# jinhojsk515/spmm

Measured on AMD Instinct MI355X. Metric: pretrain molecules/sec, higher is better.
Workload: dtype bf16; 1 GPU; SPMM pretrain step, text 12 layers (fusion at 6) + PV 6 layers, H=768, 12 heads, queue 36864, train mode (dropout 0.1), fwd+bwd+clip+AdamW+EMA; global_batch=128, seq_len=128, parallelism=dp1, schedule=eager launches on three HIP streams, packed text rows

## Files before the change

include/spmm_hip.h:

```cpp
#ifndef SPMM_HIP_H
#define SPMM_HIP_H

#include <stdint.h>

#ifdef __HIPCC__
#include <hip/hip_runtime.h>
typedef hipStream_t spmm_stream_t;
#else
typedef void* spmm_stream_t;
#endif

#ifdef __cplusplus
extern "C" {
#endif

int spmm_version(void);
const char* spmm_last_error(void);

#define SPMM_EPI_BF16 0
#define SPMM_EPI_GELU 1
#define SPMM_EPI_F32 2
#define SPMM_EPI_F32_ATOMIC 3
#define SPMM_EPI_GELU_GRAD 4
#define SPMM_EPI_F32_ACC 5
// ... 72 lines not shown
int spmm_beam_step_until(const float* logits, long ldl, int N, int k, int V, int Lmax, int F, int t, const int* t_ptr, int t_off,
                         int* tokens, float* cur_p, float* fin_p, int* fin_len, int* fin_tok, int* fin_n, unsigned char* done,
                         int* anc, int anc_ld, int* ids_out, int* parent_out, int* n_done, const int* mol, const int* rowmap,
                         int need, spmm_stream_t stream);

int spmm_beam_step_sampled(const float* logits, long ldl, int N, int k, int V, int Lmax, int F, int t, const int* t_ptr, int t_off,
                           int* tokens, float* cur_p, float* fin_p, int* fin_len, int* fin_tok, int* fin_n, unsigned char* done,
                           int* anc, int anc_ld, int* ids_out, int* parent_out, int* n_done, const int* mol, const int* rowmap,
                           const float* noise, long ldn, spmm_stream_t stream);

int spmm_gumbel_noise(const uint64_t* seed_ptr, uint64_t salt, int N, int k, int V, int Lmax, int t, const int* t_ptr, int t_off,
                      const int* mol, long mol_base, float* out, long ldo, spmm_stream_t stream);

int spmm_logit_warp(const float* lc, const float* lu, long ld, int R, int V, float w, float temperature, int top_k, float top_p,
                    int min_keep, float* out, long ldo, spmm_stream_t stream);

#define SPMM_SYNTAX_MASKED (-1e30f)
int spmm_smiles_mask(float* logits, float* logits2, long ld, int R, int V, const int* tokens, long tok_ld, int hist_rows, int k,
                     const int* mol, int Lmax, int t, const int* t_ptr, int t_off, int t_last, const int* table, int* state_out,
                     spmm_stream_t stream);

int spmm_wordpiece(const unsigned char* blob, const long* offsets, int N, int gap, const unsigned char* head, int head_len,
                   const int* table, int table_words, int max_chars, int max_pieces, int unk_id, int sep_id, int pad_id,
                   int* ids, long ld, int* lens, int* status, spmm_stream_t stream);

int spmm_sbs_step(const float* logits, long ldl, const float* noise, long ldn, int G, int W, int V, int Lmax, int t, const int* t_ptr,
                  int t_off, const float* phi_in, const float* gum_in, const unsigned char* fin_in, const int* len_in,
                  const int* tokens_in, const int* anc_in, float* phi_out, float* gum_out, unsigned char* fin_out, int* len_out,
                  int* tokens_out, int* anc_out, int anc_ld, int* ids_out, int* parent_out, int* open_out, unsigned int* ws,
                  spmm_stream_t stream);

int spmm_kv_prefill(const void* K, const void* V, long ld, long src_rows, const int* row0, const int* len, const int* dst_row, int E,
                    void* Kc, void* Vc, int R, int nH, int Lmax, spmm_stream_t stream);

int spmm_embed_ln_fwd(int mode, const int* ids, const float* word, const float* pos, const float* type0, const float* pv_x,
                      const float* pv_mask, const float* pv_w, const float* pv_b, const float* pv_cls,
                      const float* pv_masktok, int src_mod, const float* gamma, const float* beta, void* y, void* zout,
                      float* mean, float* rstd, long nseq, int L, int H, float eps, float dropout_p,
                      const uint64_t* seed_ptr, uint64_t salt, spmm_stream_t stream);
int spmm_embed_bwd(int mode, const void* dz, const int* ids, const float* pv_x, const float* pv_mask, int src_mod,
                   float* dword, float* dpos, float* dtype0, float* d_w, float* d_b, float* d_cls, float* d_masktok,
                   long nseq, int L, int H, spmm_stream_t stream);

int spmm_transpose_bf16(const void* in, long ldi, void* out, long ldo, int R, int C, int Rpad, float* colsum,
                        spmm_stream_t stream);
int spmm_cast_transpose(const float* in, void* out, void* outT, int R, int C, spmm_stream_t stream);
long spmm_cast_transpose_desc_bytes(void);
int spmm_cast_transpose_multi(const void* descs_dev, int ndesc, int total_tiles, spmm_stream_t stream);
int spmm_cast_f32_bf16(const float* in, void* out, long n, spmm_stream_t stream);
int spmm_cast_bf16_f32(const void* in, float* out, long n, spmm_stream_t stream);
int spmm_acc_rows(float* dst, long ldd, const void* src, long lds, const long* idx, long rows, int H, int atomic,
                  spmm_stream_t stream);
int spmm_gather_rows(void* dst, const void* src, const long* idx, long rows, int H, spmm_stream_t stream);

int spmm_gather_rows2(void* dst, const void* srcA, const void* srcB, const long* idx, long rows, int H, spmm_stream_t stream);
int spmm_add_rows_bf16(void* dst, const long* idx, const void* src, long rows, int H, spmm_stream_t stream);
int spmm_zero_bytes(void* p, long nbytes, spmm_stream_t stream);
int spmm_zero_rows(void* p, long rows, long row_bytes, long stride_bytes, spmm_stream_t stream);
int spmm_gelu_bwd(const void* dz, const void* pre, void* out, long n, spmm_stream_t stream);
int spmm_pack_plan(const int* mask, int B, int Lt, int M, int* lens32, int* row0_32, long* row0_64, long* rows, long* gidx2,
                   long* gidx4, long* inv, long* idx_m, int* bad, spmm_stream_t stream);
int spmm_fusion_plan(const long* neg, const int* lens32, const int* row0_32, int B, int Lt, int Lp, int M,
                     long* idx6, long* neg_rows, long* idx_top, int* small32, spmm_stream_t stream);

int spmm_l2norm_fwd(const float* x, long ldx, float* y, float* nrm, void* a3, void* w3, void* yT, long ldt, int rows, int E,
                    spmm_stream_t stream);
int spmm_l2norm_bwd(const float* dy, const float* y, const float* nrm, const float* gscale, void* dx, int rows, int E,
                    spmm_stream_t stream);
int spmm_ita_rows(const float* S, const float* SM, long ldj, int nrows, int B, int J, const float* alpha_ptr,
                  const float* temp_ptr, void* dS, long ldd, int Jpad, float* losses, int loss_slot, float* dtemp,
                  int* nan_flag, spmm_stream_t stream);
int spmm_sample_neg(const float* S, long ldj, int B, const long* forced, const uint64_t* seed_ptr, uint64_t salt, long* out,
                    long out_offset, spmm_stream_t stream);
int spmm_lm_loss(const float* logits, const float* logits_m, long ldl, const int* ids, long nseq, int L, int V,
                 const float* alpha_ptr, int* n_nonpad_ws, const float* gscale, void* dlogits, long ldd, int Vpad,
                 float* losses, int loss_slot, spmm_stream_t stream);
int spmm_s2s_loss(const float* logits, long ldl, const int* ids, const long* row_of, long rows, long nseq, int L, int V,
                  int* n_label_ws, const float* gscale, void* dlogits, long ldd, int Vpad, float* losses, int loss_slot,
                  spmm_stream_t stream);
int spmm_lm_score(const void* y, long ldy, const void* Wd, long ldw, const float* bias, const int* ids, const long* row_of, long rows,
                  long nseq, int L, int V, int H, const int* seq_row0, const int* seq_len, float* tok_lp, float* seq_lp, int* seq_n,
                  spmm_stream_t stream);
int spmm_itm_head(const void* xa, long stride_a, const void* xb, long stride_b, int H, const float* W, const float* bias,
                  int n, int B, const float* gscale, float* losses, int loss_slot, float* logits_out, void* dxa, void* dxb,
                  float* dW, float* db, int do_bwd, int x_is_f32, spmm_stream_t stream);
int spmm_task_head(const void* A, long lda, int B, int W, const float* W2, const float* b2, int C, int kind, const void* target,
                   const float* gscale, float* logits, float* loss, void* dA, long ldda, float* dW2, float* db2, int do_bwd,
                   spmm_stream_t stream);
int spmm_s2p_append(const void* y, long ldy, const float* w3, const float* b3, const float* pe_w, const float* pe_b, const float* pos,
                    const float* type0, const float* gamma, const float* beta, float eps, float* pred, long ldp, void* xcache,
                    long rows, int H, int n_props, int i, spmm_stream_t stream);
int spmm_mpm_head(const void* h, int Lp, int H, const float* w, const float* bias, const float* target, const float* mask,
                  int B, int* n_keep_ws, const float* gscale, float* losses, int loss_slot, float* pred_out, void* dh,
                  float* dw, float* db, int do_bwd, int x_is_f32, spmm_stream_t stream);
int spmm_rows_linear(const void* x, int x_is_bf16, long ldx, const float* W, const float* bias, float* out, long ldo, long rows,
                     int N, int K, int act, spmm_stream_t stream);
long spmm_sim_topk_workspace_bytes(int Q, long n, int k);
int spmm_sim_topk(const float* q, long ldq, const float* f, long ldf, long base, int Q, long n, int E, int k, float* scores, long* index,
                  int merge, const float* cut_scores, const long* cut_index, void* workspace, long workspace_bytes, spmm_stream_t stream);
int spmm_centroid_assign(const float* f, long ldf, const float* c, long ldc, long c0, long n, int Kc, int E, float* best, int* assign,
                         int merge, const int* prev, int* changed, spmm_stream_t stream);
long spmm_cluster_group_workspace_bytes(long n, int K);
int spmm_cluster_group(const int* assign, long n, int K, int* counts, long* offsets, int* members, int* outside, void* workspace,
                       long workspace_bytes, spmm_stream_t stream);
long spmm_cluster_centroids_workspace_bytes(long n, int K, int E);
int spmm_cluster_centroids(const float* f, long ldf, long n, int E, const float* best, const int* counts, const long* offsets,
// ... 21 lines not shown
```

spmm_amd/csrc/rowops.hip:

```cpp
#include "common.h"
#include <stdlib.h>
#include "../../include/spmm_hip.h"

namespace {

constexpr int MAXC = 4;

struct RowVec {
  float v[MAXC][4];
};

__device__ __forceinline__ void load_row_bf16(const bf16* __restrict__ p, int H, int lane, RowVec& r) {
#pragma unroll
  for (int i = 0; i < MAXC; ++i) {
    const int c = (lane + 64 * i) * 4;
    if (c < H) {
      const bf16x4 t = *(const bf16x4*)(p + c);
      r.v[i][0] = (float)t[0]; r.v[i][1] = (float)t[1]; r.v[i][2] = (float)t[2]; r.v[i][3] = (float)t[3];
    } else {
      r.v[i][0] = r.v[i][1] = r.v[i][2] = r.v[i][3] = 0.f;
    }
  }
}
__device__ __forceinline__ void store_row_bf16(bf16* __restrict__ p, int H, int lane, const RowVec& r) {
// ... 433 lines not shown
    const uint32_t rowkey = drop_rowkey(seed_mix(p.seed_ptr, p.salt), (uint64_t)row);
#pragma unroll
    for (int i = 0; i < MAXC; ++i) {
      const int c = (lane + 64 * i) * 4;
      if (c < p.H) {
        bool k[4];
        drop_keep4(rowkey, c, p.thresh16, k);
#pragma unroll
        for (int j = 0; j < 4; ++j) o.v[i][j] = k[j] ? o.v[i][j] * p.dscale : 0.f;
      }
    }
  }
  store_row_bf16(p.y + row * p.H, p.H, lane, o);
  if (p.zout) store_row_bf16(p.zout + row * p.H, p.H, lane, z);
  if (p.mean_o && lane == 0) { p.mean_o[row] = mean; p.rstd_o[row] = rstd; }
}

struct EmbedBwdP {
  const bf16* dz; const int* ids; const float* pv_x; const float* pv_mask; int src_mod;
  float* dword; float* dpos; float* dtype0; float* d_w; float* d_b; float* d_cls; float* d_masktok;
  long nseq; int L, H, mode;
};
__global__ __launch_bounds__(256) void embed_bwd_kernel(EmbedBwdP p) {
  const int l = blockIdx.x;
  const long s_per = (p.nseq + gridDim.y - 1) / gridDim.y;
  const long s_beg = blockIdx.y * s_per, s_end = min(p.nseq, s_beg + s_per);
  for (int c = threadIdx.x; c < p.H; c += 256) {
    float acc = 0.f, accw = 0.f, accb = 0.f, accm = 0.f;
    for (long s = s_beg; s < s_end; ++s) {
      const long row = s * p.L + l;
      const float g = (float)p.dz[row * p.H + c];
      acc += g;
      if (p.mode == 0) {
        const int id = p.ids[row];
        if (id != 0) atomicAdd(p.dword + (long)id * p.H + c, g);
      } else if (l > 0) {
        const long src = (s % p.src_mod) * (p.L - 1) + (l - 1);
        const float m = p.pv_mask[src];
        accw += g * (1.f - m) * p.pv_x[src];
        accb += g * (1.f - m);
        accm += g * m;
      }
    }
    atomicAdd(p.dpos + (long)l * p.H + c, acc);
    atomicAdd(p.dtype0 + c, acc);
    if (p.mode == 1) {
      if (l == 0) {
        atomicAdd(p.d_cls + c, acc);
      } else {
        atomicAdd(p.d_w + c, accw);
        atomicAdd(p.d_b + c, accb);
        atomicAdd(p.d_masktok + c, accm);
      }
    }
  }
}

__global__ __launch_bounds__(256) void transpose_bf16_kernel(const bf16* __restrict__ in, long ldi, bf16* __restrict__ out,
                                                             long ldo, int R, int C, int Rpad, float* __restrict__ colsum) {
  __shared__ bf16 tile[64][66];
  const int r0 = blockIdx.y * 64, c0 = blockIdx.x * 64;
  const int tx = threadIdx.x & 63, ty = threadIdx.x >> 6;
  float cs = 0.f;
#pragma unroll
  for (int i = 0; i < 16; ++i) {
    const int r = r0 + ty * 16 + i, c = c0 + tx;
    const bf16 v = (r < R && c < C) ? in[(long)r * ldi + c] : (bf16)0.f;
    tile[ty * 16 + i][tx] = v;
    cs += (float)v;
  }
  if (colsum) {
    __shared__ float part[4][64];
    part[ty][tx] = cs;
    __syncthreads();
    if (ty == 0 && c0 + tx < C) atomicAdd(colsum + c0 + tx, part[0][tx] + part[1][tx] + part[2][tx] + part[3][tx]);
  } else {
    __syncthreads();
  }
#pragma unroll
  for (int i = 0; i < 16; ++i) {
    const int c = c0 + ty * 16 + i, r = r0 + tx;
    if (c < C && r < Rpad) out[(long)c * ldo + r] = tile[tx][ty * 16 + i];
  }
}

__global__ __launch_bounds__(256) void cast_transpose_kernel(const float* __restrict__ in, bf16* __restrict__ out,
                                                             bf16* __restrict__ outT, int R, int C) {
  __shared__ bf16 tile[64][66];
  const int r0 = blockIdx.y * 64, c0 = blockIdx.x * 64;
  const int tx = threadIdx.x & 63, ty = threadIdx.x >> 6;
#pragma unroll
  for (int i = 0; i < 16; ++i) {
    const int r = r0 + ty * 16 + i, c = c0 + tx;
    bf16 v = (bf16)0.f;
    if (r < R && c < C) {
      v = (bf16)in[(long)r * C + c];
      if (out) out[(long)r * C + c] = v;
    }
    tile[ty * 16 + i][tx] = v;
  }
  __syncthreads();
  if (outT) {
#pragma unroll
    for (int i = 0; i < 16; ++i) {
      const int c = c0 + ty * 16 + i, r = r0 + tx;
      if (c < C && r < R) outT[(long)c * R + r] = tile[tx][ty * 16 + i];
// ... 148 lines not shown
  return SPMM_OK;
}

extern "C" int spmm_embed_ln_fwd(int mode, const int* ids, const float* word, const float* pos, const float* type0,
                                 const float* pv_x, const float* pv_mask, const float* pv_w, const float* pv_b,
                                 const float* pv_cls, const float* pv_masktok, int src_mod, const float* gamma,
                                 const float* beta, void* y, void* zout, float* mean, float* rstd, long nseq, int L, int H,
                                 float eps, float dropout_p, const uint64_t* seed_ptr, uint64_t salt, hipStream_t stream) {
  SPMM_CHECK_SHAPE(nseq > 0 && L > 0 && H > 0 && H % 4 == 0 && H <= 1024, "spmm_embed_ln_fwd: nseq=%ld L=%d H=%d (need 0 < H <= 1024, H%%4==0)", nseq, L, H);
  SPMM_CHECK_SHAPE(mode >= 0 && mode <= 2, "spmm_embed_ln_fwd: unknown mode %d", mode);
  SPMM_CHECK_SHAPE(pos && type0 && gamma && beta && y, "spmm_embed_ln_fwd: null pos / type0 / gamma / beta / y");
  SPMM_CHECK_SHAPE((mean == nullptr) == (rstd == nullptr), "spmm_embed_ln_fwd: mean and rstd come together");
  SPMM_CHECK_SHAPE(mode == 0 ? (ids && word) : mode == 2 ? (pv_x != nullptr) : (pv_x && pv_mask && pv_w && pv_b && pv_cls && pv_masktok && src_mod > 0),
                   "spmm_embed_ln_fwd: missing inputs for mode %d", mode);
  SPMM_CHECK_SHAPE(dropout_p == 0.f || seed_ptr, "spmm_embed_ln_fwd: dropout needs a device seed");
  EmbedP p = {};
  p.ids = ids; p.word = word; p.pos = pos; p.type0 = type0; p.pv_x = pv_x; p.pv_mask = pv_mask; p.pv_w = pv_w; p.pv_b = pv_b;
  p.pv_cls = pv_cls; p.pv_masktok = pv_masktok; p.src_mod = src_mod; p.gamma = gamma; p.beta = beta; p.y = (bf16*)y;
  p.zout = (bf16*)zout; p.mean_o = mean; p.rstd_o = rstd; p.nseq = nseq; p.L = L; p.H = H; p.mode = mode; p.eps = eps;
  p.thresh16 = (uint32_t)(dropout_p * 65536.f + 0.5f); p.dscale = 1.f / (1.f - dropout_p); p.seed_ptr = seed_ptr; p.salt = salt;
  hipLaunchKernelGGL(embed_ln_fwd_kernel, dim3((nseq * L + 3) / 4), dim3(256), 0, stream, p);
  SPMM_LAUNCH_CHECK("spmm_embed_ln_fwd");
  return SPMM_OK;
}

extern "C" int spmm_embed_step_ln_fwd(const int* ids, int pos_index, const int* pos_ptr, const float* word, const float* pos, const float* type0,
                                      const float* gamma, const float* beta, void* y, long rows, int H, float eps,
                                      hipStream_t stream) {
  SPMM_CHECK_SHAPE(rows > 0 && pos_index >= 0 && H % 4 == 0 && H <= 1024, "spmm_embed_step_ln_fwd: rows=%ld pos=%d H=%d", rows, pos_index, H);
  SPMM_CHECK_SHAPE(ids && word && pos && type0 && gamma && beta && y, "spmm_embed_step_ln_fwd: null argument");
  EmbedP p = {};
  p.ids = ids; p.word = word; p.pos = pos; p.type0 = type0; p.gamma = gamma; p.beta = beta; p.y = (bf16*)y;
  p.nseq = rows; p.L = 1; p.H = H; p.mode = 0; p.eps = eps; p.pos0 = pos_index; p.pos_ptr = pos_ptr; p.dscale = 1.f;
  hipLaunchKernelGGL(embed_ln_fwd_kernel, dim3((rows + 3) / 4), dim3(256), 0, stream, p);
  SPMM_LAUNCH_CHECK("spmm_embed_step_ln_fwd");
  return SPMM_OK;
}

extern "C" int spmm_embed_bwd(int mode, const void* dz, const int* ids, const float* pv_x, const float* pv_mask, int src_mod,
                              float* dword, float* dpos, float* dtype0, float* d_w, float* d_b, float* d_cls,
                              float* d_masktok, long nseq, int L, int H, hipStream_t stream) {
  SPMM_CHECK_SHAPE(nseq > 0 && L > 0 && H > 0, "spmm_embed_bwd: nseq=%ld L=%d H=%d", nseq, L, H);
  SPMM_CHECK_SHAPE(mode == 0 || mode == 1, "spmm_embed_bwd: mode %d (0 = text, 1 = PV; inputs_embeds has no backward)", mode);
  SPMM_CHECK_SHAPE(dz && dpos && dtype0, "spmm_embed_bwd: null dz / dpos / dtype0");
  SPMM_CHECK_SHAPE(mode != 0 || (ids && dword), "spmm_embed_bwd: mode 0 needs ids and dword");
  SPMM_CHECK_SHAPE(mode != 1 || (pv_x && pv_mask && d_w && d_b && d_cls && d_masktok), "spmm_embed_bwd: mode 1 needs pv_x, pv_mask, d_w, d_b, d_cls and d_masktok");
  SPMM_CHECK_SHAPE(mode != 1 || src_mod > 0, "spmm_embed_bwd: mode 1 needs src_mod > 0, got src_mod=%d", src_mod);
  EmbedBwdP p = {(const bf16*)dz, ids, pv_x, pv_mask, src_mod, dword, dpos, dtype0, d_w, d_b, d_cls, d_masktok, nseq, L, H, mode};
  hipLaunchKernelGGL(embed_bwd_kernel, dim3(L, nseq >= 32 ? 16 : 1), dim3(256), 0, stream, p);
  SPMM_LAUNCH_CHECK("spmm_embed_bwd");
  return SPMM_OK;
}

namespace {
__global__ __launch_bounds__(256) void segment_sum_kernel(const bf16* __restrict__ src, const int* __restrict__ start,
                                                          const int* __restrict__ list, bf16* __restrict__ out, long W) {
  const int u = blockIdx.y;
  const long c = ((long)blockIdx.x * 256 + threadIdx.x) * 8;
  if (c >= W) return;
  const int k0 = start[u], k1 = start[u + 1];
  float acc[8] = {0.f, 0.f, 0.f, 0.f, 0.f, 0.f, 0.f, 0.f};
  for (int k = k0; k < k1; ++k) {
    const bf16x8 v = *(const bf16x8*)(src + (long)list[k] * W + c);
#pragma unroll
    for (int e = 0; e < 8; ++e) acc[e] += (float)v[e];
  }
  bf16x8 o;
#pragma unroll
  for (int e = 0; e < 8; ++e) o[e] = (bf16)acc[e];
  *(bf16x8*)(out + (long)u * W + c) = o;
}
}

extern "C" int spmm_segment_sum_bf16(const void* src, const int* start, const int* list, void* out, int U, long W, hipStream_t stream) {
  SPMM_CHECK_SHAPE(U > 0 && U <= 65535 && W > 0 && W % 8 == 0, "spmm_segment_sum_bf16: U=%d W=%ld (W %% 8 == 0)", U, W);
  SPMM_CHECK_SHAPE(src && start && list && out, "spmm_segment_sum_bf16: null src / start / list / out");
  hipLaunchKernelGGL(segment_sum_kernel, dim3((unsigned)((W / 8 + 255) / 256), U), dim3(256), 0, stream, (const bf16*)src, start, list,
                     (bf16*)out, W);
  SPMM_LAUNCH_CHECK("spmm_segment_sum_bf16");
  return SPMM_OK;
}

extern "C" int spmm_transpose_bf16(const void* in, long ldi, void* out, long ldo, int R, int C, int Rpad, float* colsum,
                                   hipStream_t stream) {
  SPMM_CHECK_SHAPE(R > 0 && C > 0 && Rpad >= R && ldo >= Rpad, "spmm_transpose_bf16: R=%d C=%d Rpad=%d ldo=%ld", R, C, Rpad, ldo);
  SPMM_CHECK_SHAPE(ldi >= C, "spmm_transpose_bf16: ldi=%ld is shorter than a row of C=%d", ldi, C);
  SPMM_CHECK_SHAPE(in && out, "spmm_transpose_bf16: null in / out");
  hipLaunchKernelGGL(transpose_bf16_kernel, dim3((C + 63) / 64, (Rpad + 63) / 64), dim3(256), 0, stream, (const bf16*)in, ldi,
                     (bf16*)out, ldo, R, C, Rpad, colsum);
  SPMM_LAUNCH_CHECK("spmm_transpose_bf16");
  return SPMM_OK;
}

extern "C" int spmm_cast_transpose(const float* in, void* out, void* outT, int R, int C, hipStream_t stream) {
  SPMM_CHECK_SHAPE(R > 0 && C > 0, "spmm_cast_transpose: R=%d C=%d", R, C);
  SPMM_CHECK_SHAPE(in && (out || outT), "spmm_cast_transpose: null in, or neither out nor outT");
  hipLaunchKernelGGL(cast_transpose_kernel, dim3((C + 63) / 64, (R + 63) / 64), dim3(256), 0, stream, in, (bf16*)out, (bf16*)outT, R, C);
  SPMM_LAUNCH_CHECK("spmm_cast_transpose");
  return SPMM_OK;
}

extern "C" long spmm_cast_transpose_desc_bytes(void) { return sizeof(CtDesc); }
extern "C" int spmm_cast_transpose_multi(const void* descs_dev, int ndesc, int total_tiles, hipStream_t stream) {
  SPMM_CHECK_SHAPE(ndesc > 0 && total_tiles > 0, "spmm_cast_transpose_multi: ndesc=%d tiles=%d", ndesc, total_tiles);
  hipLaunchKernelGGL(cast_transpose_multi_kernel, dim3(total_tiles), dim3(256), 0, stream, (const CtDesc*)descs_dev, ndesc);
  SPMM_LAUNCH_CHECK("spmm_cast_transpose_multi");
// ... 37 lines not shown
```

spmm_amd/ops.py:

```python
import ctypes
import os

import torch

from ._lib import lib

EPI_BF16, EPI_GELU, EPI_F32, EPI_F32_ATOMIC, EPI_GELU_GRAD, EPI_F32_ACC, EPI_GELU_DERIV, EPI_MUL = range(8)
BF16 = torch.bfloat16


_DRY_RUN = False
_dry_log = []


def _p(t):
    return None if t is None else ctypes.c_void_p(t.data_ptr())


def _st():
    if _DRY_RUN:
        return None
    return ctypes.c_void_p(torch.cuda.current_stream().cuda_stream)


# ... 169 lines not shown

def ln_bwd(dy, z, mean, rstd, gamma, dz, *, dy2=None, dx=None, dgamma=None, dbeta=None, dropout_p=0.0, seed=None, salt=0,
           drop_on_dy=False, dxsum=None, rows_dev=None, beta_from_y=None):
    rows, H = dy.shape
    _call("spmm_ln_bwd", _p(dy), _p(dy2), _p(z), _p(mean), _p(rstd), _p(gamma), _p(dz), _p(dx), _p(dgamma), _p(dbeta),
               rows, H, float(dropout_p), _p(seed), salt, int(drop_on_dy), _p(dxsum), _p(rows_dev), _p(beta_from_y), _st())
    return dz


def embed_ln_fwd(mode, y, *, nseq, L, H, pos, type0, gamma, beta, ids=None, word=None, pv_x=None, pv_mask=None, pv_w=None,
                 pv_b=None, pv_cls=None, pv_masktok=None, src_mod=1, zout=None, mean=None, rstd=None, eps=1e-12,
                 dropout_p=0.0, seed=None, salt=0):
    _call("spmm_embed_ln_fwd", mode, _p(ids), _p(word), _p(pos), _p(type0), _p(pv_x), _p(pv_mask), _p(pv_w), _p(pv_b),
               _p(pv_cls), _p(pv_masktok), src_mod, _p(gamma), _p(beta), _p(y), _p(zout), _p(mean), _p(rstd), nseq, L, H,
               float(eps), float(dropout_p), _p(seed), salt, _st())
    return y


def embed_bwd(mode, dz, *, nseq, L, H, dpos, dtype0, ids=None, dword=None, pv_x=None, pv_mask=None, src_mod=1, d_w=None,
              d_b=None, d_cls=None, d_masktok=None):
    _call("spmm_embed_bwd", mode, _p(dz), _p(ids), _p(pv_x), _p(pv_mask), src_mod, _p(dword), _p(dpos), _p(dtype0),
               _p(d_w), _p(d_b), _p(d_cls), _p(d_masktok), nseq, L, H, _st())


def transpose_bf16(x, out, *, Rpad=None, colsum=None):
    R, C = x.shape
    Rpad = out.shape[1] if Rpad is None else Rpad
    _call("spmm_transpose_bf16", _p(x), _row_stride(x), _p(out), _row_stride(out), R, C, Rpad, _p(colsum), _st())
    return out


def cast_transpose(w32, out, outT):
    R, C = w32.shape
    _call("spmm_cast_transpose", _p(w32), _p(out), _p(outT), R, C, _st())


def cast_transpose_multi(descs_dev, ndesc, total_tiles):
    _call("spmm_cast_transpose_multi", _p(descs_dev), ndesc, total_tiles, _st())


def cast_f32_bf16(x, out):
    _call("spmm_cast_f32_bf16", _p(x), _p(out), x.numel(), _st())
    return out


def cast_bf16_f32(x, out):
    _call("spmm_cast_bf16_f32", _p(x), _p(out), x.numel(), _st())
    return out


def acc_rows(dst, src, *, idx=None, atomic=False):
    rows, H = src.shape
    _call("spmm_acc_rows", _p(dst), _row_stride(dst), _p(src), _row_stride(src), _p(idx), rows, H, int(atomic), _st())


def gather_rows(dst, src, idx):
    rows, H = dst.shape
    _call("spmm_gather_rows", _p(dst), _p(src), _p(idx), rows, H, _st())
    return dst


SRC_B = 1 << 40


def gather_rows2(dst, srcA, idx, srcB=None):
    rows, H = dst.shape
    assert idx.dtype == torch.int64 and idx.numel() >= rows and dst.is_contiguous() and srcA.is_contiguous() and (srcB is None or srcB.is_contiguous())
    assert dst.dtype == BF16 and srcA.dtype == BF16 and srcA.shape[1] == H and (srcB is None or (srcB.dtype == BF16 and srcB.shape[1] == H))
    _call("spmm_gather_rows2", _p(dst), _p(srcA), _p(srcB), _p(idx), rows, H, _st())
    return dst


def add_rows_bf16(dst, idx, src):
    rows, H = src.shape
    assert dst.dtype == BF16 and src.dtype == BF16 and idx.dtype == torch.int64 and dst.is_contiguous() and src.is_contiguous() and dst.shape[1] == H
    _call("spmm_add_rows_bf16", _p(dst), _p(idx), _p(src), rows, H, _st())
    return dst


def zero_(t):
    n = t.numel() * t.element_size()
    if n == 0:
        return t
    if not t.is_contiguous():
        es = t.element_size()
        if t.dim() == 2 and t.stride(1) == 1 and (t.shape[1] * es) % 16 == 0 and (t.stride(0) * es) % 16 == 0 and t.data_ptr() % 16 == 0:
            _call("spmm_zero_rows", _p(t), t.shape[0], t.shape[1] * es, t.stride(0) * es, _st())
            return t
        return t.zero_()
    if n % 16 or t.data_ptr() % 16:
        return t.zero_()
    _call("spmm_zero_bytes", _p(t), n, _st())
    return t


def gelu_bwd(dz, pre, out=None):
    assert dz.dtype == BF16 and pre.dtype == BF16 and dz.is_contiguous() and pre.is_contiguous() and dz.shape == pre.shape
    out = torch.empty_like(dz) if out is None else out
    _call("spmm_gelu_bwd", _p(dz), _p(pre), _p(out), dz.numel(), _st())
    return out


def pack_plan(mask32, M, bad):
    B, Lt = mask32.shape
    dev = mask32.device
    alloc = torch.zeros if _DRY_RUN else torch.empty
# ... 533 lines not shown
```

spmm_amd/options.py:

```python
from __future__ import annotations

import dataclasses
import os
from dataclasses import dataclass

_ENV = {
    "pack_text": ("SPMM_PACK_TEXT", lambda s: s != "0"),
    "cls_only_top": ("SPMM_CLS_ONLY_TOP", lambda s: s != "0"),
    "multi_stream": ("SPMM_STREAMS", lambda s: s != "1"),
    "wgrad_stream": ("SPMM_WGRAD_STREAM", lambda s: s != "0"),
    "pv_wgrad_inline": ("SPMM_PV_WGRAD_INLINE", int),
    "ln_from_y": ("SPMM_LN_FROM_Y", lambda s: s != "0"),
    "resid_fp32": ("SPMM_RESID_FP32", lambda s: s == "1"),
    "fused_xattn": ("SPMM_FUSED_XATTN", lambda s: {"0": "off", "1": "all"}.get(s, s)),
    "grad_overlap": ("SPMM_GRAD_OVERLAP", lambda s: s != "0"),
    "grad_wire": ("SPMM_GRAD_WIRE", str),
    "nt_under_comm": ("SPMM_NT_UNDER_COMM", str),
    "force_dist": ("SPMM_FORCE_DIST", lambda s: s == "1"),
    "dp_four_streams": ("SPMM_DP_FOUR_STREAMS", lambda s: s != "0"),
    "probe_streams": ("SPMM_PROBE_STREAMS", lambda s: s != "0"),
    "schedule_check": ("SPMM_SCHEDULE_CHECK", lambda s: s != "0"),
}


@dataclass
class EngineOptions:
    pack_text: bool = True
    cls_only_top: bool = True
    multi_stream: bool = True
    wgrad_stream: bool = True
    pv_wgrad_inline: int = 4
    ln_from_y: bool = True
    fused_xattn: str = "nograd"
    resid_fp32: bool = False
    grad_overlap: bool = True
    grad_wire: str = "fp32"
    nt_under_comm: str = "auto"
    force_dist: bool = False
    dp_four_streams: bool = True
    schedule_check: bool = True
    probe_streams: bool = False

    @classmethod
    def from_env(cls, **overrides) -> "EngineOptions":
        kw = {}
        for field, (var, parse) in _ENV.items():
            if var in os.environ:
                kw[field] = parse(os.environ[var])
        kw.update(overrides)
        o = cls(**kw)
        if isinstance(o.fused_xattn, bool):
            o.fused_xattn = "all" if o.fused_xattn else "off"
        if o.fused_xattn not in ("off", "nograd", "all"):
            raise ValueError(f"fused_xattn must be off, nograd or all, not {o.fused_xattn!r}")
        if o.grad_wire not in ("fp32", "bf16"):
            raise ValueError(f"grad_wire must be fp32 or bf16, not {o.grad_wire!r}")
        if o.nt_under_comm not in ("tiles", "persistent", "auto"):
            raise ValueError(f"nt_under_comm must be tiles, persistent or auto, not {o.nt_under_comm!r}")
        return o

    def replace(self, **kw) -> "EngineOptions":
        return dataclasses.replace(self, **kw)
```

spmm_amd/step.py:

```python
from __future__ import annotations

from typing import Callable, Optional, Tuple

import torch

from . import ops, streams
from .engine import STREAM_TOKENS_MAX, BF, LOSS_ITA, LOSS_ITM, LOSS_MLM, LOSS_MPM, Batch, Engine, Group, KVSource, SelfKV, _ceil


class PretrainStep(Engine):
    def _s6_forward_cls(self, B, Lt, M, pk, mask32, neg, y1, y2, prop_embeds, text_embeds, save):
        cfg = self.cfg
        ct = cfg.text
        H, Lp, f, n = ct.hidden_size, cfg.n_props + 1, ct.fusion_layer, ct.num_hidden_layers
        fp = ops.fusion_plan(neg, pk, Lp)
        o_tp = 3 * B * Lp
        o_lm = o_tp + 2 * M
        o_12 = o_lm + B * Lt
        o_8 = o_12 + B * Lp
        Rcap = fp["Rcap"]
        X6 = ops.gather_rows2(self._new(Rcap, H), y1, fp["idx6"], y2)
        src_pv = KVSource(prop_embeds.view(B * Lp, H), B, Lp).preset(4 * B, fp["start_p"], fp["list_p"])
        src_text = KVSource(text_embeds, B, Lt, row0=pk["row0"], length=pk["len"], pack_idx=pk["rows"]).preset(4 * B, fp["start_t"], fp["list_t"])
        ar = fp["ar"]
# ... 257 lines not shown

        if aux is not None:
            aux.update(prop_embeds=prop_embeds, text_embeds=text_embeds, prop_embeds_m=prop_embeds_m, text_embeds_m=text_embeds_m,
                       prop_feat=feats["property_proj"][0], text_feat=feats["text_proj"][0], prop_feat_m=feats["property_proj_m"][0],
                       text_feat_m=feats["text_proj_m"][0], sim_i2t=S_text[:B], sim_t2i=S_prop[B:2 * B], sim_i2t_m=S_text[2 * B:3 * B],
                       vl_output=vl_logits, mlm_output=logits.view(B, Lt, -1)[:, :-1], logits_m=logits_m.view(B, Lt, -1)[:, :-1],
                       pred=pred, prop_neg_idx=neg[:B], text_neg_idx=neg[B:], mpm_mask=mpm_mask,
                       prop_embeds_causal=prop_embeds_causal)
        if save:
            self.tape = dict(B=B, Lt=Lt, pk=pk, M=M, Mn=Mn, src_text=src_text, src_pv=src_pv, neg_rows=neg_rows, cls_text=cls_text, itm_text=itm_text,
                             prop=prop, mpm_mask=mpm_mask, ids32=ids32, ids2=ids2, esv1=esv1, g1=g1, tape1=tape1,
                             esv2=esv2, g2=g2, tape2=tape2, feats=feats, dfeat=dfeat, neg=neg, g6=g6, tape6=tape6, ypv=ypv_h,
                             ytext=ytext, logits=logits, logits_m=logits_m, lmsv=lmsv, mpmsv=mpmsv, S6=S6 if cls_top else None)
        return self.losses[:4]

    def backward(self):
        T = self.tape
        if T is None:
            raise RuntimeError("backward() without a taped forward()")
        self.pre_backward_wait()
        cfg, P = self.cfg, self.P
        ct, cp = cfg.text, cfg.prop
        H, E, Lp, f, n = ct.hidden_size, cfg.embed_dim, cfg.n_props + 1, ct.fusion_layer, ct.num_hidden_layers
        B, Lt = T["B"], T["Lt"]
        gs = self.gscale
        scratch = self.loss_scratch
        pk, M = T["pk"], T["M"]
        S6 = T["S6"]
        if S6 is not None:
            dYtop = self._new(S6["ntop"], H)
            dY_mpm, dY_lm = dYtop[6 * B + B * Lt:], dYtop[6 * B:6 * B + B * Lt]
        else:
            nt6 = T["ytext"].shape[0]
            dY6 = self._zeros(4 * B * Lp + nt6, H)
            dYpv, dYtext = dY6[:4 * B * Lp], dY6[4 * B * Lp:]
            dY_mpm, dY_lm = dYpv[3 * B * Lp:], dYtext[nt6 - B * Lt:]

        dmln = self._new(B * Lp, H)
        ops.mpm_head(T["mpmsv"].ln.y, Lp, H, P.w("property_mtr_head.3.weight"), P.w("property_mtr_head.3.bias"), T["prop"], T["mpm_mask"], B=B,
                     ws=self.icount[4:8], losses=scratch, slot=LOSS_MPM, dh=dmln, dw=P.g("property_mtr_head.3.weight"),
                     db=P.g("property_mtr_head.3.bias"), gscale=gs[1:2])
        dmpre = self._transform_bwd(T["mpmsv"], dmln)
        ops.gemm_nt(dmpre, self._wT("property_mtr_head.0", P.w("property_mtr_head.0.weight")), dY_mpm)

        V = ct.vocab_size
        dlogits = self._new(B * Lt, _ceil(V, 64))
        ops.lm_loss(T["logits"], T["logits_m"], T["ids32"], nseq=B, L=Lt, V=V, alpha=self.alpha, ws=self.icount[0:4], losses=scratch,
                    slot=LOSS_MLM, dlogits=dlogits, gscale=gs[0:1])
        self.lm_head_bwd("text_encoder.", ct, T["lmsv"], dlogits, out=dY_lm)

        neg_p, neg_t = T["neg"][:B], T["neg"][B:]
        d_pe = self._zeros(B, Lp * H, dtype=torch.float32)
        d_te = self._zeros(M + 1, H, dtype=torch.float32)
        if S6 is not None:
            ytop = S6["ytop"]
            ops.itm_head(ytop[:3 * B], H, ytop[3 * B:6 * B], H, H, P.w("itm_head.weight"), P.w("itm_head.bias"), n=3 * B, B=B, losses=scratch,
                         slot=LOSS_ITM, dxa=dYtop[:3 * B], dxb=dYtop[3 * B:6 * B], dW=P.g("itm_head.weight"), db=P.g("itm_head.bias"), gscale=gs[3:4])
            dX6 = self._s6_backward_cls(T, dYtop, d_pe, d_te)
            dXpv = dX6[:3 * B * Lp].view(3 * B, Lp * H)
            dXt = dX6[S6["o_tp"]:S6["o_lm"]]
            ops.acc_rows(d_pe, dXpv[0:B])
            ops.acc_rows(d_pe, dXpv[B:2 * B], idx=neg_p, atomic=True)
            ops.acc_rows(d_pe, dXpv[2 * B:3 * B])
            ops.acc_rows(d_te[:M], dXt[:M])
            ops.acc_rows(d_te[:M], dXt[M:2 * M])
            ops.acc_rows(d_te, dX6[S6["o_8"]:], idx=S6["fp"]["neg_rows"], atomic=True)
            dXt_lm, dX12 = dX6[S6["o_lm"]:S6["o_12"]], dX6[S6["o_12"]:S6["o_8"]]
        else:
            ditm = self._new(3 * B, H)
            ops.itm_head(T["ypv"], Lp * H, T["itm_text"], H, H, P.w("itm_head.weight"), P.w("itm_head.bias"), n=3 * B, B=B, losses=scratch,
                         slot=LOSS_ITM, dxa=dYpv, dxb=ditm, dW=P.g("itm_head.weight"), db=P.g("itm_head.bias"), gscale=gs[3:4])
            dYtext.index_copy_(0, T["cls_text"], ditm)
            dX6 = self.stack_bwd("text_encoder.bert.", ct, range(f, n), T["tape6"], dY6, T["g6"],
                                 dkv_acc={id(T["src_text"]): d_te[:M], id(T["src_pv"]): d_pe.view(B * Lp, H)})
            dXpv, dXt = dX6[:4 * B * Lp].view(4 * B, Lp * H), dX6[4 * B * Lp:]
            ops.acc_rows(d_pe, dXpv[0:B])
            ops.acc_rows(d_pe, dXpv[B:2 * B], idx=neg_p, atomic=True)
            ops.acc_rows(d_pe, dXpv[2 * B:3 * B])
            if pk:
                ops.acc_rows(d_te[:M], dXt[:M])
                ops.acc_rows(d_te[:M], dXt[M:2 * M])
                nr = T["neg_rows"]
                ops.acc_rows(d_te, dXt[2 * M:2 * M + T["Mn"]], idx=torch.where(nr < M, nr, torch.full_like(nr, -1)), atomic=True)
            else:
                dte, dxt = d_te[:M].view(B, Lt * H), dXt.view(4 * B, Lt * H)
                ops.acc_rows(dte, dxt[0:B])
                ops.acc_rows(dte, dxt[B:2 * B])
                ops.acc_rows(dte, dxt[2 * B:3 * B], idx=neg_t, atomic=True)
            dXt_lm, dX12 = dXt[nt6 - B * Lt:], dXpv[3 * B:].reshape(B * Lp, H)

        for k, proj in enumerate(("property_proj", "text_proj")):
            feat, nrm, cls = T["feats"][proj]
            dproj = self._new(B, E)
            ops.l2norm_bwd(T["dfeat"][k * B:(k + 1) * B], feat, nrm, dproj, gscale=gs[2:3])
            self._wgrad(dproj, cls, P.g(proj + ".weight"), P.g(proj + ".bias"))
            dcls = self._new(B, H)
            ops.gemm_nt(dproj, self._wT(proj, P.w(proj + ".weight")), dcls)
            if k == 0:
                ops.acc_rows(d_pe[:, :H], dcls)
            elif pk:
                ops.acc_rows(d_te, dcls, idx=pk["row0_64"])
            else:
                ops.acc_rows(d_te[:M].view(B, Lt * H)[:, :H], dcls)
        ops.axpy_scalar(P.g("temp").view(1), self.dtemp_ita, scale_ptr=gs[2:3])

        side = self._fork()
        with self._on(side):
            dY2 = self._new(M + B * Lt, H)
            ops.cast_f32_bf16(d_te[:M].view(-1), dY2[:M].view(-1))
            dY2[M:].copy_(dXt_lm)
            dX2 = self.stack_bwd("text_encoder.bert.", ct, range(0, f), T["tape2"], dY2, T["g2"])
            if pk:
                dX2 = ops.gather_rows2(self._new(2 * B * Lt, H), dX2, pk["inv"])
            dz2 = self._embed_ln_bwd("text_encoder.bert.", ct, T["esv2"], dX2)
            tp = "text_encoder.bert.embeddings."
            ops.embed_bwd(0, dz2, nseq=2 * B, L=Lt, H=H, dpos=P.g(tp + "position_embeddings.weight"),
                          dtype0=P.g(tp + "token_type_embeddings.weight"), ids=T["ids2"], dword=P.g(tp + "word_embeddings.weight"))

        dY1 = self._new(2 * B * Lp, H)
        ops.cast_f32_bf16(d_pe.view(-1), dY1[:B * Lp].view(-1))
        dY1[B * Lp:].copy_(dX12)
        nl1 = cp.num_hidden_layers
        k1 = min(max(int(self.opt.pv_wgrad_inline), 0), nl1) if side is not None else 0
        dX1 = self.stack_bwd("property_encoder.", cp, range(k1, nl1), T["tape1"][k1:], dY1, T["g1"])
        wa, self.wgrad_async = self.wgrad_async, False
        dX1 = self.stack_bwd("property_encoder.", cp, range(0, k1), T["tape1"][:k1], dX1, T["g1"])
        self.wgrad_async = wa
        dz1 = self._embed_ln_bwd("property_encoder.", cp, T["esv1"], dX1)
        pp = "property_encoder.embeddings."
        ops.embed_bwd(1, dz1, nseq=2 * B, L=Lp, H=H, dpos=P.g(pp + "position_embeddings.weight"),
                      dtype0=P.g(pp + "token_type_embeddings.weight"), pv_x=T["prop"], pv_mask=T["mpm_mask"], src_mod=B,
                      d_w=P.g("property_embed.weight"), d_b=P.g("property_embed.bias"), d_cls=P.g("property_cls"),
                      d_masktok=P.g("property_mask"))
        self._join(side)
        self.end_backward()
```

Baseline: 2456 molecules/s.

## Fuse fusion-stage gradient scatter-adds, cast and copy into hub_finish gather kernel

Replaces the chain of acc_rows calls (some atomic scatter-adds over negative-sample rows), the CLS-gradient adds, the fp32-to-bf16 cast and the row copy with one gather-style kernel per encoder. For each output row it sums the base fp32 gradient, identity terms, list-indexed negative-sample terms and position-0 CLS terms, then writes bf16 directly. This removes several launches, the fp32 read-modify-write traffic and the atomics. In exchange it needs precomputed inverse lists (start/list) and a per-term loop per row. It is enabled by default through the hub_gather option.

```diff
diff --git a/include/spmm_hip.h b/include/spmm_hip.h
--- a/include/spmm_hip.h
+++ b/include/spmm_hip.h
@@ -148,6 +148,9 @@
 int spmm_acc_rows(float* dst, long ldd, const void* src, long lds, const long* idx, long rows, int H, int atomic,
                   spmm_stream_t stream);
 int spmm_gather_rows(void* dst, const void* src, const long* idx, long rows, int H, spmm_stream_t stream);
+long spmm_hub_term_bytes(void);
+int spmm_hub_finish(const float* base, void* out, const int* unit_row0, const int* unit_len, int U, int L, long hub_rows, int H,
+                    const void* terms, int nterms, const void* copy_src, long copy_rows, spmm_stream_t stream);
 
 int spmm_gather_rows2(void* dst, const void* srcA, const void* srcB, const long* idx, long rows, int H, spmm_stream_t stream);
 int spmm_add_rows_bf16(void* dst, const long* idx, const void* src, long rows, int H, spmm_stream_t stream);
diff --git a/spmm_amd/csrc/rowops.hip b/spmm_amd/csrc/rowops.hip
--- a/spmm_amd/csrc/rowops.hip
+++ b/spmm_amd/csrc/rowops.hip
@@ -509,6 +509,91 @@
         atomicAdd(p.d_b + c, accb);
         atomicAdd(p.d_masktok + c, accm);
       }
+    }
+  }
+}
+
+struct HubTerm {
+  const bf16* src; long src_rows;
+  const int* start; const int* list; const int* crow0; const int* rows_dev;
+  int kind, lo, hi, pad_;
+};
+constexpr int HUB_MAX_TERMS = 6;
+struct HubP {
+  const float* base; bf16* out; const int* urow0; const int* ulen; const bf16* copy_src;
+  long hub_rows, copy_rows;
+  int U, L, H, nterms, ny;
+  HubTerm t[HUB_MAX_TERMS];
+};
+__device__ __forceinline__ void hub_add(float (&a)[2][8], const bf16* __restrict__ row, int H, int lane) {
+#pragma unroll
+  for (int i = 0; i < 2; ++i) {
+    const int c = (lane + 64 * i) * 8;
+    if (c < H) {
+      const bf16x8 v = *(const bf16x8*)(row + c);
+#pragma unroll
+      for (int e = 0; e < 8; ++e) a[i][e] += (float)v[e];
+    }
+  }
+}
+__global__ __launch_bounds__(256) void hub_finish_kernel(HubP p) {
+  const int lane = threadIdx.x & 63, wave = threadIdx.x >> 6, H = p.H;
+  const long hub_blocks = (long)p.U * p.ny;
+  if ((long)blockIdx.x >= hub_blocks) {
+    const long r = ((long)blockIdx.x - hub_blocks) * 4 + wave;
+    if (r >= p.copy_rows) return;
+#pragma unroll
+    for (int i = 0; i < 2; ++i) {
+      const int c = (lane + 64 * i) * 8;
+      if (c < H) *(bf16x8*)(p.out + (p.hub_rows + r) * H + c) = *(const bf16x8*)(p.copy_src + r * H + c);
+    }
+    return;
+  }
+  const int u = (int)(blockIdx.x / p.ny), l = (int)(blockIdx.x % p.ny) * 4 + wave;
+  const int len = p.ulen ? p.ulen[u] : p.L;
+  if (l >= len || l >= p.L) return;
+  const long row = (p.urow0 ? (long)p.urow0[u] : (long)u * p.L) + l;
+  if (row < 0 || row >= p.hub_rows) return;
+  float a[2][8];
+#pragma unroll
+  for (int i = 0; i < 2; ++i) {
+    const int c = (lane + 64 * i) * 8;
+#pragma unroll
+    for (int e = 0; e < 8; ++e) a[i][e] = 0.f;
+    if (c < H) {
+      const f32x4 x = *(const f32x4*)(p.base + row * H + c), y = *(const f32x4*)(p.base + row * H + c + 4);
+#pragma unroll
+      for (int e = 0; e < 4; ++e) { a[i][e] = x[e]; a[i][4 + e] = y[e]; }
+    }
+  }
+  for (int k = 0; k < p.nterms; ++k) {
+    const HubTerm& t = p.t[k];
+    if (t.kind == 0) {
+      if (row < t.src_rows) hub_add(a, t.src + row * H, H, lane);
+    } else if (t.kind == 2) {
+      if (l == 0 && u < t.src_rows) hub_add(a, t.src + (long)u * H, H, lane);
+    } else {
+      long lim = t.src_rows;
+      if (t.rows_dev) { const long rd = *t.rows_dev; lim = rd < lim ? rd : lim; }
+      const int q1 = t.start[u + 1];
+      for (int q = t.start[u]; q < q1; ++q) {
+        const int e = t.list[q];
+        if (e < t.lo || e >= t.hi) continue;
+        const int j = e - t.lo;
+        const long cr = (t.crow0 ? (long)t.crow0[j] : (long)j * p.L) + l;
+        if (cr < 0 || cr >= lim) continue;
+        hub_add(a, t.src + cr * H, H, lane);
+      }
+    }
+  }
+#pragma unroll
+  for (int i = 0; i < 2; ++i) {
+    const int c = (lane + 64 * i) * 8;
+    if (c < H) {
+      bf16x8 o;
+#pragma unroll
+      for (int e = 0; e < 8; ++e) o[e] = (bf16)a[i][e];
+      *(bf16x8*)(p.out + row * H + c) = o;
     }
   }
 }
@@ -763,6 +848,33 @@
   return SPMM_OK;
 }
 
+extern "C" long spmm_hub_term_bytes(void) { return sizeof(HubTerm); }
+extern "C" int spmm_hub_finish(const float* base, void* out, const int* unit_row0, const int* unit_len, int U, int L, long hub_rows, int H,
+                               const void* terms, int nterms, const void* copy_src, long copy_rows, hipStream_t stream) {
+  SPMM_CHECK_SHAPE(U > 0 && L > 0 && hub_rows > 0 && H > 0 && H % 8 == 0 && H <= 1024, "spmm_hub_finish: U=%d L=%d hub_rows=%ld H=%d (need H%%8==0, H<=1024)",
+                   U, L, hub_rows, H);
+  SPMM_CHECK_SHAPE(base && out, "spmm_hub_finish: null base / out");
+  SPMM_CHECK_SHAPE((unit_row0 == nullptr) == (unit_len == nullptr), "spmm_hub_finish: unit_row0 and unit_len come together");
+  SPMM_CHECK_SHAPE(unit_row0 || (long)U * L <= hub_rows, "spmm_hub_finish: %d units of %d rows exceed hub_rows=%ld", U, L, hub_rows);
+  SPMM_CHECK_SHAPE(nterms >= 0 && nterms <= HUB_MAX_TERMS && (nterms == 0 || terms), "spmm_hub_finish: nterms=%d (at most %d, with a table)", nterms, HUB_MAX_TERMS);
+  SPMM_CHECK_SHAPE(copy_rows >= 0 && (copy_rows == 0 || copy_src), "spmm_hub_finish: copy_rows=%ld needs copy_src", copy_rows);
+  HubP p = {};
+  p.base = base; p.out = (bf16*)out; p.urow0 = unit_row0; p.ulen = unit_len; p.copy_src = (const bf16*)copy_src;
+  p.hub_rows = hub_rows; p.copy_rows = copy_rows;
+  p.U = U; p.L = L; p.H = H; p.nterms = nterms; p.ny = (L + 3) / 4;
+  for (int k = 0; k < nterms; ++k) {
+    const HubTerm& t = ((const HubTerm*)terms)[k];
+    SPMM_CHECK_SHAPE(t.kind >= 0 && t.kind <= 2 && t.src && t.src_rows > 0, "spmm_hub_finish: term %d: kind=%d src_rows=%ld (or null src)", k, t.kind, t.src_rows);
+    SPMM_CHECK_SHAPE(t.kind != 1 || (t.start && t.list && t.hi > t.lo), "spmm_hub_finish: term %d: a by-list term needs start, list and lo < hi", k);
+    p.t[k] = t;
+  }
+  const long blocks = (long)U * p.ny + (copy_rows + 3) / 4;
+  SPMM_CHECK_SHAPE(blocks < (1l << 31), "spmm_hub_finish: %ld workgroups", blocks);
+  hipLaunchKernelGGL(hub_finish_kernel, dim3((unsigned)blocks), dim3(256), 0, stream, p);
+  SPMM_LAUNCH_CHECK("spmm_hub_finish");
+  return SPMM_OK;
+}
+
 namespace {
 __global__ __launch_bounds__(256) void segment_sum_kernel(const bf16* __restrict__ src, const int* __restrict__ start,
                                                           const int* __restrict__ list, bf16* __restrict__ out, long W) {
diff --git a/spmm_amd/ops.py b/spmm_amd/ops.py
--- a/spmm_amd/ops.py
+++ b/spmm_amd/ops.py
@@ -245,6 +245,42 @@
 def acc_rows(dst, src, *, idx=None, atomic=False):
     rows, H = src.shape
     _call("spmm_acc_rows", _p(dst), _row_stride(dst), _p(src), _row_stride(src), _p(idx), rows, H, int(atomic), _st())
+
+
+class _HubTerm(ctypes.Structure):
+    _fields_ = [("src", ctypes.c_void_p), ("src_rows", ctypes.c_long), ("start", ctypes.c_void_p), ("list", ctypes.c_void_p),
+                ("crow0", ctypes.c_void_p), ("rows_dev", ctypes.c_void_p), ("kind", ctypes.c_int), ("lo", ctypes.c_int), ("hi", ctypes.c_int),
+                ("pad", ctypes.c_int)]
+
+
+HUB_IDENTITY, HUB_BY_LIST, HUB_POS0 = range(3)
+_hub_layout_ok = False
+
+
+def hub_term(kind, src, *, start=None, lst=None, lo=0, hi=0, crow0=None, rows_dev=None):
+    assert src.dtype == BF16 and src.dim() == 2 and src.is_contiguous()
+    assert all(t is None or (t.dtype == torch.int32 and t.is_contiguous()) for t in (start, lst, crow0, rows_dev))
+    return (kind, src, start, lst, lo, hi, crow0, rows_dev)
+
+
+def hub_finish(base, out, terms, *, U, L, unit_row0=None, unit_len=None, copy_src=None):
+    R, H = base.shape
+    nc = 0 if copy_src is None else copy_src.shape[0]
+    assert base.dtype == torch.float32 and base.is_contiguous() and out.dtype == BF16 and out.is_contiguous() and out.shape == (R + nc, H)
+    assert copy_src is None or (copy_src.dtype == BF16 and copy_src.is_contiguous() and copy_src.shape[1] == H)
+    assert all(t is None or (t.dtype == torch.int32 and t.is_contiguous() and t.numel() >= U) for t in (unit_row0, unit_len))
+    assert all(t[1].shape[1] == H for t in terms)
+    tab = (_HubTerm * max(len(terms), 1))()
+    for d, (kind, src, start, lst, lo, hi, crow0, rows_dev) in zip(tab, terms):
+        d.src, d.src_rows, d.kind, d.lo, d.hi = src.data_ptr(), src.shape[0], kind, lo, hi
+        d.start, d.list, d.crow0, d.rows_dev = (None if t is None else t.data_ptr() for t in (start, lst, crow0, rows_dev))
+    global _hub_layout_ok
+    if not (_DRY_RUN or _hub_layout_ok):
+        assert ctypes.sizeof(_HubTerm) == lib().cdll.spmm_hub_term_bytes()
+        _hub_layout_ok = True
+    _call("spmm_hub_finish", _p(base), _p(out), _p(unit_row0), _p(unit_len), U, L, R, H, ctypes.c_void_p(ctypes.addressof(tab)), len(terms),
+          _p(copy_src), nc, _st())
+    return out
 
 
 def gather_rows(dst, src, idx):
diff --git a/spmm_amd/options.py b/spmm_amd/options.py
--- a/spmm_amd/options.py
+++ b/spmm_amd/options.py
@@ -11,6 +11,7 @@
     "wgrad_stream": ("SPMM_WGRAD_STREAM", lambda s: s != "0"),
     "pv_wgrad_inline": ("SPMM_PV_WGRAD_INLINE", int),
     "ln_from_y": ("SPMM_LN_FROM_Y", lambda s: s != "0"),
+    "hub_gather": ("SPMM_HUB_GATHER", lambda s: s != "0"),
     "resid_fp32": ("SPMM_RESID_FP32", lambda s: s == "1"),
     "fused_xattn": ("SPMM_FUSED_XATTN", lambda s: {"0": "off", "1": "all"}.get(s, s)),
     "grad_overlap": ("SPMM_GRAD_OVERLAP", lambda s: s != "0"),
@@ -31,6 +32,7 @@
     wgrad_stream: bool = True
     pv_wgrad_inline: int = 4
     ln_from_y: bool = True
+    hub_gather: bool = True
     fused_xattn: str = "nograd"
     resid_fp32: bool = False
     grad_overlap: bool = True
diff --git a/spmm_amd/step.py b/spmm_amd/step.py
--- a/spmm_amd/step.py
+++ b/spmm_amd/step.py
@@ -333,6 +333,7 @@
         neg_p, neg_t = T["neg"][:B], T["neg"][B:]
         d_pe = self._zeros(B, Lp * H, dtype=torch.float32)
         d_te = self._zeros(M + 1, H, dtype=torch.float32)
+        hub = S6 is not None and self.opt.hub_gather
         if S6 is not None:
             ytop = S6["ytop"]
             ops.itm_head(ytop[:3 * B], H, ytop[3 * B:6 * B], H, H, P.w("itm_head.weight"), P.w("itm_head.bias"), n=3 * B, B=B, losses=scratch,
@@ -340,12 +341,22 @@
             dX6 = self._s6_backward_cls(T, dYtop, d_pe, d_te)
             dXpv = dX6[:3 * B * Lp].view(3 * B, Lp * H)
             dXt = dX6[S6["o_tp"]:S6["o_lm"]]
-            ops.acc_rows(d_pe, dXpv[0:B])
-            ops.acc_rows(d_pe, dXpv[B:2 * B], idx=neg_p, atomic=True)
-            ops.acc_rows(d_pe, dXpv[2 * B:3 * B])
-            ops.acc_rows(d_te[:M], dXt[:M])
-            ops.acc_rows(d_te[:M], dXt[M:2 * M])
-            ops.acc_rows(d_te, dX6[S6["o_8"]:], idx=S6["fp"]["neg_rows"], atomic=True)
+            fp = S6["fp"]
+            if hub:
+                BLp = B * Lp
+                terms_pe = [ops.hub_term(ops.HUB_IDENTITY, dX6[:BLp]),
+                            ops.hub_term(ops.HUB_BY_LIST, dX6[BLp:2 * BLp], start=fp["start_p"], lst=fp["list_p"], lo=B, hi=2 * B),
+                            ops.hub_term(ops.HUB_IDENTITY, dX6[2 * BLp:3 * BLp])]
+                terms_te = [ops.hub_term(ops.HUB_IDENTITY, dXt[:M]), ops.hub_term(ops.HUB_IDENTITY, dXt[M:2 * M]),
+                            ops.hub_term(ops.HUB_BY_LIST, dX6[S6["o_8"]:], start=fp["start_t"], lst=fp["list_t"], lo=2 * B, hi=3 * B,
+                                         crow0=fp["row0_8"], rows_dev=fp["mn_dev"])]
+            else:
+                ops.acc_rows(d_pe, dXpv[0:B])
+                ops.acc_rows(d_pe, dXpv[B:2 * B], idx=neg_p, atomic=True)
+                ops.acc_rows(d_pe, dXpv[2 * B:3 * B])
+                ops.acc_rows(d_te[:M], dXt[:M])
+                ops.acc_rows(d_te[:M], dXt[M:2 * M])
+                ops.acc_rows(d_te, dX6[S6["o_8"]:], idx=fp["neg_rows"], atomic=True)
             dXt_lm, dX12 = dX6[S6["o_lm"]:S6["o_12"]], dX6[S6["o_12"]:S6["o_8"]]
         else:
             ditm = self._new(3 * B, H)
@@ -377,7 +388,9 @@
             self._wgrad(dproj, cls, P.g(proj + ".weight"), P.g(proj + ".bias"))
             dcls = self._new(B, H)
             ops.gemm_nt(dproj, self._wT(proj, P.w(proj + ".weight")), dcls)
-            if k == 0:
+            if hub:
+                (terms_pe, terms_te)[k].append(ops.hub_term(ops.HUB_POS0, dcls))
+            elif k == 0:
                 ops.acc_rows(d_pe[:, :H], dcls)
             elif pk:
                 ops.acc_rows(d_te, dcls, idx=pk["row0_64"])
@@ -388,8 +401,11 @@
         side = self._fork()
         with self._on(side):
             dY2 = self._new(M + B * Lt, H)
-            ops.cast_f32_bf16(d_te[:M].view(-1), dY2[:M].view(-1))
-            dY2[M:].copy_(dXt_lm)
+            if hub:
+                ops.hub_finish(d_te[:M], dY2, terms_te, U=B, L=Lt, unit_row0=pk["row0"], unit_len=pk["len"], copy_src=dXt_lm)
+            else:
+                ops.cast_f32_bf16(d_te[:M].view(-1), dY2[:M].view(-1))
+                dY2[M:].copy_(dXt_lm)
             dX2 = self.stack_bwd("text_encoder.bert.", ct, range(0, f), T["tape2"], dY2, T["g2"])
             if pk:
                 dX2 = ops.gather_rows2(self._new(2 * B * Lt, H), dX2, pk["inv"])
@@ -399,8 +415,11 @@
                           dtype0=P.g(tp + "token_type_embeddings.weight"), ids=T["ids2"], dword=P.g(tp + "word_embeddings.weight"))
 
         dY1 = self._new(2 * B * Lp, H)
-        ops.cast_f32_bf16(d_pe.view(-1), dY1[:B * Lp].view(-1))
-        dY1[B * Lp:].copy_(dX12)
+        if hub:
+            ops.hub_finish(d_pe.view(B * Lp, H), dY1, terms_pe, U=B, L=Lp, copy_src=dX12)
+        else:
+            ops.cast_f32_bf16(d_pe.view(-1), dY1[:B * Lp].view(-1))
+            dY1[B * Lp:].copy_(dX12)
         nl1 = cp.num_hidden_layers
         k1 = min(max(int(self.opt.pv_wgrad_inline), 0), nl1) if side is not None else 0
         dX1 = self.stack_bwd("property_encoder.", cp, range(k1, nl1), T["tape1"][k1:], dY1, T["g1"])
```

Result: no change. 2466 molecules/s (median of 6 runs) (+0.4%).
